# Regenerator/dpf-nets

Hardware: AMD Instinct MI355X
Metric: points/sec through 14-layer flow + Chamfer, B=32 N=2048 (higher is better)
Workload: dtype f16x3 MFMA operands, fp32 accumulate/points; 1 GPU; configs[1]: airplane autoencoder shapes, B=32 N=2048 per GPU: 14 coupling layers (first 14 of LocalCondRNVPDecoder(n_flows=5)), direct/eval-BN, + nn_distance both directions + CD reduction; clouds_per_gpu=32, points_per_cloud=2048, hidden=64, latent=128, global_clouds=32, per_layer_lists=False, launch=hipGraph replay, 10 step(s) per graph, steps_in_flight=1, settle_steps=400, parallelism=clouds sharded, no collective, sclk_mhz=2199, chamfer_impl=auto (matrix-core filtered exact search at this size)

## Files before the change

dpf_nets_amd/csrc/chamfer_mfma.hip:

```cpp
#include <hip/hip_runtime.h>
#include <limits.h>
#include <stdint.h>
#include <stdlib.h>

#include "dpf_hip.h"
#include "lds_attr.h"
#include "zero_fill.h"
#include "nn_refscan.h"

#pragma clang fp contract(off)

namespace {

typedef __bf16 bf16x8 __attribute__((ext_vector_type(8)));
typedef float f32x16 __attribute__((ext_vector_type(16)));
typedef uint32_t u32x4 __attribute__((ext_vector_type(4)));

constexpr int CT = 64;
constexpr int PROW = 100;
constexpr int SCH = 32;
constexpr int WCAP = SCH * 64 / 8;
constexpr int NNM_PTS = CT * 1024, NNM_LISTS = NNM_PTS + CT * PROW * 4;
__host__ __device__ constexpr int nnm_lds_bytes(int qw) { return NNM_LISTS + qw * SCH * 64 + qw * WCAP * 2; }

__device__ __forceinline__ uint32_t f2u(float x) { return __builtin_bit_cast(uint32_t, x); }
__device__ __forceinline__ float u2f(uint32_t x) { return __builtin_bit_cast(float, x); }
__device__ __forceinline__ uint32_t bf16_rne(float x) {
    const uint32_t u = f2u(x);
    return (u + 0x7FFFu + ((u >> 16) & 1u)) >> 16;
}
__device__ __forceinline__ void split2(float x, uint32_t &hi, uint32_t &lo) {
    const uint32_t h = f2u(x) & 0xFFFF0000u;
    hi = h >> 16;
    lo = bf16_rne(x - u2f(h));
}

__host__ __device__ inline int tiles_of(int n) { return (n + 31) / 32; }

__device__ __forceinline__ void cand_coord(float c, uint32_t &w0, uint32_t &w1) {
    uint32_t hi, lo;
    split2(c, hi, lo);
    w0 = hi | (hi << 16);
    w1 = lo | (lo << 16);
}
__device__ __forceinline__ void cand_fragment(float x, float y, float z, bool live, uint4 &h0, uint4 &h1) {
    cand_coord(x, h0.x, h0.y);
    cand_coord(y, h0.z, h0.w);
    cand_coord(z, h1.x, h1.y);
    const float w = (x * x + y * y) + z * z;
    const float ww = live ? w : 3.0e38f;
    const uint32_t wh = f2u(ww) & 0xFFFF0000u;
    const float r1 = ww - u2f(wh);
    const uint32_t wm = f2u(r1) & 0xFFFF0000u;
    const float r2 = r1 - u2f(wm);
    h1.z = (wh >> 16) | (live ? wm : 0u);
    h1.w = live ? bf16_rne(r2) : 0u;
}
__device__ __forceinline__ uint4 query_fragment(float x, float y, float z, int h) {
    uint32_t ah, al, bh, bl;
    split2(-2.0f * (h ? z : x), ah, al);
    split2(-2.0f * y, bh, bl);
    uint4 o;
    o.x = ah | (al << 16); o.y = o.x;
    o.z = h ? 0x3F803F80u : (bh | (bl << 16));
    o.w = h ? 0x00003F80u : o.z;
    return o;
}

struct MDir {
    const float *q, *c;
    float *dist;
    int *idx;
    int nq, nc;
    long qstride, cstride;
};
struct MArgs { MDir d[2]; int pn2; float *part; unsigned *ticket; float *cd; };

__device__ __forceinline__ f32x16 mfma(uint4 a, uint4 b) {
    const f32x16 z = {0.f, 0.f, 0.f, 0.f, 0.f, 0.f, 0.f, 0.f, 0.f, 0.f, 0.f, 0.f, 0.f, 0.f, 0.f, 0.f};
    return __builtin_amdgcn_mfma_f32_32x32x16_bf16(__builtin_bit_cast(bf16x8, a), __builtin_bit_cast(bf16x8, b), z, 0, 0, 0);
}
__device__ __forceinline__ float tile_min(const f32x16 &s) {
    float m = fminf(fminf(s[0], s[1]), s[2]);
    m = fminf(fminf(m, s[3]), s[4]);   m = fminf(fminf(m, s[5]), s[6]);
    m = fminf(fminf(m, s[7]), s[8]);   m = fminf(fminf(m, s[9]), s[10]);
    m = fminf(fminf(m, s[11]), s[12]); m = fminf(fminf(m, s[13]), s[14]);
    return fminf(fminf(m, s[15]), s[0]);
}
__device__ __forceinline__ float dist3(float cx, float cy, float cz, float qx, float qy, float qz) {
    const float dx = cx - qx, dy = cy - qy, dz = cz - qz;
    return (dx * dx + dy * dy) + dz * dz;
}
template <class P>
__device__ __forceinline__ void exact_tile(P cp, int nc, int t, int tl, int h, float qx, float qy, float qz,
                                           float &best, int &bidx) {
    float d[16];
#pragma unroll
    for (int g = 0; g < 4; ++g) {
        const float *row = cp + (size_t)tl * PROW + 8 * g + 4 * h;
        const float4 vx = *(const float4 *)row, vy = *(const float4 *)(row + 32), vz = *(const float4 *)(row + 64);
        d[4 * g + 0] = dist3(vx.x, vy.x, vz.x, qx, qy, qz); d[4 * g + 1] = dist3(vx.y, vy.y, vz.y, qx, qy, qz);
        d[4 * g + 2] = dist3(vx.z, vy.z, vz.z, qx, qy, qz); d[4 * g + 3] = dist3(vx.w, vy.w, vz.w, qx, qy, qz);
    }
    float m = fminf(fminf(d[0], d[1]), d[2]);
#pragma unroll
    for (int r = 3; r < 15; r += 2) m = fminf(fminf(m, d[r]), d[r + 1]);
    m = fminf(m, d[15]);
    if (m <= best) {
        int kmin = INT_MAX;
#pragma unroll
        for (int r = 15; r >= 0; --r) {
            const int k = t * 32 + 8 * (r >> 2) + 4 * h + (r & 3);
            kmin = (d[r] == m && k < nc) ? k : kmin;
        }
        const bool better = kmin != INT_MAX && (m < best || kmin < bidx);
        best = better ? m : best;
        bidx = better ? kmin : bidx;
    }
}

template <class P>
__device__ __forceinline__ void exact_tile_mk(P cp, int nc, int t, int tl, int h, float qx, float qy, float qz, float &m, int &kmin) {
    float d[16];
#pragma unroll
    for (int g = 0; g < 4; ++g) {
        const float *row = cp + (size_t)tl * PROW + 8 * g + 4 * h;
        const float4 vx = *(const float4 *)row, vy = *(const float4 *)(row + 32), vz = *(const float4 *)(row + 64);
        d[4 * g + 0] = dist3(vx.x, vy.x, vz.x, qx, qy, qz); d[4 * g + 1] = dist3(vx.y, vy.y, vz.y, qx, qy, qz);
        d[4 * g + 2] = dist3(vx.z, vy.z, vz.z, qx, qy, qz); d[4 * g + 3] = dist3(vx.w, vy.w, vz.w, qx, qy, qz);
    }
    m = fminf(fminf(d[0], d[1]), d[2]);
#pragma unroll
    for (int r = 3; r < 15; r += 2) m = fminf(fminf(m, d[r]), d[r + 1]);
    m = fminf(m, d[15]);
    kmin = INT_MAX;
#pragma unroll
    for (int r = 15; r >= 0; --r) {
        const int k = t * 32 + 8 * (r >> 2) + 4 * h + (r & 3);
        kmin = (d[r] == m && k < nc) ? k : kmin;
    }
}

typedef __attribute__((address_space(3))) void lds_void;
typedef __attribute__((address_space(1))) const void glb_void;

template <int QW>
__global__ __launch_bounds__(QW * 64) void nnm_kernel(MArgs args) {
    extern __shared__ __attribute__((aligned(16))) uint8_t lds[];
    uint4 *sfrag = (uint4 *)lds;
    float *spts = (float *)(lds + NNM_PTS);
    unsigned char *qtile = (unsigned char *)(lds + NNM_LISTS);
    __shared__ float s_r2[QW];
    const bool pairwise = args.pn2 > 0;
    const int dir = pairwise ? (int)(blockIdx.z & 1) : (int)blockIdx.z;
    const MDir A = args.d[dir];
    const int pi = pairwise ? (int)(blockIdx.z >> 1) : 0, pj = (int)blockIdx.y;
    const int bi = pairwise ? 0 : (int)blockIdx.y;
    const int nq = A.nq, nc = A.nc;
    const bool sums = args.part != nullptr;
    const size_t part_at = pairwise ? (((size_t)pi * args.pn2 + pj) * 2 + dir) * gridDim.x + blockIdx.x
                                    : ((size_t)bi * 2 + dir) * gridDim.x + blockIdx.x;
    const size_t unit = pairwise ? (size_t)pi * args.pn2 + pj : (size_t)bi;
    auto publish = [&](float t) {
        if (args.ticket == nullptr) { args.part[part_at] = t; return; }
        __hip_atomic_store(&args.part[part_at], t, __ATOMIC_RELAXED, __HIP_MEMORY_SCOPE_AGENT);
        asm volatile("s_waitcnt vmcnt(0)" ::: "memory");
        const unsigned nwg2 = 2u * gridDim.x;
        const unsigned old = __hip_atomic_fetch_add(&args.ticket[unit], 1u, __ATOMIC_RELAXED, __HIP_MEMORY_SCOPE_AGENT);
        if (old == nwg2 - 1) {
            const float *p = args.part + unit * nwg2;
            float s1 = 0.f, s2 = 0.f;
            for (unsigned x = 0; x < gridDim.x; ++x) {
                s1 += __hip_atomic_load(&p[x], __ATOMIC_RELAXED, __HIP_MEMORY_SCOPE_AGENT);
                s2 += __hip_atomic_load(&p[gridDim.x + x], __ATOMIC_RELAXED, __HIP_MEMORY_SCOPE_AGENT);
            }
            args.cd[unit] = s1 / (float)args.d[0].nq + s2 / (float)args.d[1].nq;
            __hip_atomic_store(&args.ticket[unit], 0u, __ATOMIC_RELAXED, __HIP_MEMORY_SCOPE_AGENT);
        }
    };
    if ((int)blockIdx.x * QW * 32 >= nq) {
        if (sums && threadIdx.x == 0) publish(0.f);
        return;
    }
    const int tid = threadIdx.x, lane = tid & 63, h = lane >> 5;
    const int wave = __builtin_amdgcn_readfirstlane(tid >> 6);
    const int qt = blockIdx.x * QW + wave;
    const int nqt = tiles_of(nq), nct = tiles_of(nc);
    const bool wave_live = qt < nqt;
    const size_t qcloud = pairwise ? (size_t)(dir == 0 ? pi : pj) * A.qstride : (size_t)bi * A.qstride;
    const size_t ccloud = pairwise ? (size_t)(dir == 0 ? pj : pi) * A.cstride : (size_t)bi * A.cstride;
    const float *__restrict__ cpts = A.c + ccloud;
    const int j = qt * 32 + (lane & 31);
    const float *qsrc = A.q + qcloud + (size_t)min(j, nq - 1) * 3;
    const float qx = qsrc[0], qy = qsrc[1], qz = qsrc[2];
    float mux, muy, muz;
    {
        const float *src = cpts + (size_t)min(lane, nc - 1) * 3;
        mux = src[0]; muy = src[1]; muz = src[2];
        for (int d = 32; d > 0; d >>= 1) { mux += __shfl_xor(mux, d); muy += __shfl_xor(muy, d); muz += __shfl_xor(muz, d); }
        mux *= 0.015625f; muy *= 0.015625f; muz *= 0.015625f;
    }
    const float qcx = qx - mux, qcy = qy - muy, qcz = qz - muz;
    const uint4 bq = query_fragment(qcx, qcy, qcz, h);
    const float INF_ = __builtin_inff();
    float r2 = j < nq ? (qcx * qcx + qcy * qcy) + qcz * qcz : 0.f;
    r2 = nn_not_finite(r2) ? INF_ : r2;
    if (nct > CT)
        for (int p = tid; p < nc; p += QW * 64) {
            const float *src = cpts + (size_t)p * 3;
            const float x = src[0] - mux, y = src[1] - muy, z = src[2] - muz;
            const float cn = (x * x + y * y) + z * z;
            r2 = nn_not_finite(cn) ? INF_ : fmaxf(r2, cn);
        }
    float tau = 0.f;
    bool slow = false;

    unsigned short *wl = (unsigned short *)(lds + NNM_LISTS + QW * SCH * 64) + (size_t)wave * WCAP;
    uint2 *res = (uint2 *)(qtile + (size_t)wave * SCH * 64);
    float smin = __builtin_inff();
    float best = __builtin_inff();
    int bidx = INT_MAX;
    const int npass = (nct + CT - 1) / CT;
    for (int pass = 0; pass < npass; ++pass) {
        const int t0 = pass * CT, tn = min(CT, nct - t0);
        if (pass > 0) __syncthreads();
        int tidp = tid;
        asm volatile("" : "+v"(tidp));
#pragma unroll
        for (int k = 0; k < CT * 32 / (QW * 64); ++k) {
            const int pl = tidp + k * QW * 64, t = pl >> 5, i = pl & 31, p = t0 * 32 + pl;
            if (t < tn) {
                const bool live = p < nc;
                float x = 0.f, y = 0.f, z = 0.f;
                if (live) { const float *src = cpts + (size_t)p * 3; x = src[0]; y = src[1]; z = src[2]; }
                uint4 f0, f1;
                const float cx = live ? x - mux : 0.f, cy = live ? y - muy : 0.f, cz = live ? z - muz : 0.f;
                cand_fragment(cx, cy, cz, live, f0, f1);
                sfrag[t * 64 + i] = f0;
                sfrag[t * 64 + 32 + i] = f1;
                spts[t * PROW + i] = live ? x : 3.0e38f; spts[t * PROW + 32 + i] = live ? y : 3.0e38f; spts[t * PROW + 64 + i] = live ? z : 3.0e38f;
                if (pass == 0) {
                    const float cn = (cx * cx + cy * cy) + cz * cz;
                    r2 = nn_not_finite(cn) ? INF_ : fmaxf(r2, cn);
                }
            }
        }
        if (pass == 0) {
            for (int d = 32; d > 0; d >>= 1) r2 = fmaxf(r2, __shfl_xor(r2, d));
            if (lane == 0) s_r2[wave] = r2;
        }
        __syncthreads();
        if (pass == 0) {
            float m = s_r2[0];
#pragma unroll
            for (int w = 1; w < QW; ++w) m = fmaxf(m, s_r2[w]);
            tau = m * 2.44140625e-4f;
            if (nn_not_finite(m)) { slow = true; break; }
        }
        if (wave_live) {
            for (int c0 = 0; c0 < tn; c0 += SCH) {
                const int cn = min(SCH, tn - c0);
                float mt[SCH];
                if (cn == SCH) {
                    const uint4 *fr = sfrag + c0 * 64 + lane;
                    if constexpr (QW < 16) {
                        uint4 fa = fr[0], fb = fr[64];
                        f32x16 a = mfma(fa, bq);
                        fa = fr[2 * 64];
#pragma unroll
                        for (int u = 0; u < SCH; u += 2) {
                            const f32x16 b = mfma(fb, bq);
                            if (u + 3 < SCH) fb = fr[(u + 3) * 64];
                            __builtin_amdgcn_sched_barrier(0);
                            mt[u] = tile_min(a);
                            __builtin_amdgcn_sched_barrier(0);
                            if (u + 2 < SCH) {
                                a = mfma(fa, bq);
                                if (u + 4 < SCH) fa = fr[(u + 4) * 64];
                            }
                            __builtin_amdgcn_sched_barrier(0);
                            mt[u + 1] = tile_min(b);
                            __builtin_amdgcn_sched_barrier(0);
                        }
                    } else {
                        f32x16 a = mfma(fr[0], bq);
#pragma unroll
                        for (int u = 0; u < SCH; u += 2) {
                            const f32x16 b = mfma(fr[(u + 1) * 64], bq);
                            __builtin_amdgcn_sched_barrier(0);
                            mt[u] = tile_min(a);
                            __builtin_amdgcn_sched_barrier(0);
                            if (u + 2 < SCH) a = mfma(fr[(u + 2) * 64], bq);
                            __builtin_amdgcn_sched_barrier(0);
                            mt[u + 1] = tile_min(b);
                            __builtin_amdgcn_sched_barrier(0);
                        }
                    }
                } else {
                    auto frag = [&](int u) { return sfrag[(c0 + min(u, cn - 1)) * 64 + lane]; };
                    f32x16 a = mfma(frag(0), bq);
#pragma unroll
                    for (int u = 0; u < SCH; u += 2) {
                        const f32x16 b = mfma(frag(u + 1), bq);
                        __builtin_amdgcn_sched_barrier(0);
                        mt[u] = tile_min(a);
                        __builtin_amdgcn_sched_barrier(0);
                        if (u + 2 < SCH) a = mfma(frag(u + 2), bq);
                        __builtin_amdgcn_sched_barrier(0);
                        mt[u + 1] = tile_min(b);
                        __builtin_amdgcn_sched_barrier(0);
                    }
                }
                float cm = fminf(fminf(mt[0], mt[1]), mt[2]);
#pragma unroll
                for (int u = 3; u + 1 < SCH; u += 2) cm = fminf(fminf(cm, mt[u]), mt[u + 1]);
                cm = fminf(cm, mt[SCH - 1]);
                smin = fminf(smin, cm);
                const float thr = fminf(smin, __shfl_xor(smin, 32)) + tau;
                unsigned smask = 0;
#pragma unroll
                for (int u = 0; u < SCH; ++u)
                    asm("v_cmp_le_f32 vcc, %1, %2\n\tv_addc_co_u32 %0, vcc, %0, %0, vcc" : "+v"(smask) : "v"(mt[u]), "v"(thr) : "vcc");
                if (cn < SCH) smask &= ~0u << (SCH - cn);
                const int nsurv = __builtin_popcount(smask);
                int smax = nsurv;
                for (int d = 32; d > 0; d >>= 1) smax = max(smax, __shfl_xor(smax, d));
                smax = __builtin_amdgcn_readfirstlane(smax);
                int off = nsurv;
#pragma unroll
                for (int d = 1; d < 64; d <<= 1) { const int v = __shfl_up(off, d); off += lane >= d ? v : 0; }
                const int W = __builtin_amdgcn_readlane(off, 63);
                off -= nsurv;
                if (W <= WCAP) {
                    {
                        unsigned mk = smask;
                        for (int e = 0; e < smax; ++e) {
                            if (mk != 0) wl[off + e] = (unsigned short)((lane << 8) | (SCH - 1 - __builtin_ctz(mk)));
                            mk &= mk - 1;
                        }
                    }
                    __builtin_amdgcn_fence(__ATOMIC_RELEASE, "wavefront");
                    __builtin_amdgcn_wave_barrier();
                    for (int i0 = 0; i0 < W; i0 += 64) {
                        const int i = i0 + lane;
                        const unsigned item = wl[min(i, W - 1)];
                        const int sl = (int)(item >> 8), tl = c0 + (int)(item & 255u);
                        const float sx = __shfl(qx, sl), sy = __shfl(qy, sl), sz = __shfl(qz, sl);
                        float m; int k;
                        exact_tile_mk(spts, nc, t0 + tl, tl, sl >> 5, sx, sy, sz, m, k);
                        if (i < W) res[i] = make_uint2(__float_as_uint(m), (unsigned)k);
                    }
                    __builtin_amdgcn_fence(__ATOMIC_RELEASE, "wavefront");
                    __builtin_amdgcn_wave_barrier();
                    for (int e = 0; e < smax; ++e) {
                        if (e < nsurv) {
                            const uint2 r = res[off + e];
                            const float m = __uint_as_float(r.x);
                            const int k = (int)r.y;
                            const bool better = k != INT_MAX && (m < best || (m == best && k < bidx));
                            best = better ? m : best;
                            bidx = better ? k : bidx;
                        }
                    }
                    __builtin_amdgcn_fence(__ATOMIC_RELEASE, "wavefront");
                    __builtin_amdgcn_wave_barrier();
                } else {
                    unsigned mk = smask;
                    for (int e = 0; e < smax; ++e) {
                        const bool take = mk != 0;
                        const int tl = c0 + (take ? SCH - 1 - __builtin_ctz(mk) : 0);
                        mk &= mk - 1;
                        float b2 = best; int i2 = bidx;
                        exact_tile(spts, nc, t0 + tl, tl, h, qx, qy, qz, b2, i2);
                        if (take) { best = b2; bidx = i2; }
                    }
                }
            }
        }
    }
    if (slow && wave_live)
        nn_reference_scan(cpts, nc, qx, qy, qz, best, bidx);
    if (!wave_live && !sums) return;
    const float od = __shfl_xor(best, 32);
    const int oi = __shfl_xor(bidx, 32);
    if (od < best || (od == best && oi < bidx)) { best = od; bidx = oi; }
    int tid_out = threadIdx.x;
    asm volatile("" : "+v"(tid_out));
    const int j_out = (blockIdx.x * QW + (tid_out >> 6)) * 32 + (tid_out & 31);
    if (!pairwise) {
        if (wave_live && h == 0 && j_out < nq) {
            A.dist[(size_t)bi * nq + j_out] = best;
            A.idx[(size_t)bi * nq + j_out] = bidx;
        }
        if (!sums) return;
    }
    float sum = (wave_live && h == 0 && j_out < nq) ? best : 0.f;
    for (int d = 16; d > 0; d >>= 1) sum += __shfl_xor(sum, d);
    __syncthreads();
    if (lane == 0) s_r2[wave] = sum;
    __syncthreads();
    if (tid == 0) {
        float t = s_r2[0];
#pragma unroll
        for (int w = 1; w < QW; ++w) t += s_r2[w];
        publish(t);
    }
}

__global__ __launch_bounds__(64) void nnm_surrogate_kernel(const float *__restrict__ q, int nq, const float *__restrict__ c, int nc,
                                                           float *__restrict__ s, float *__restrict__ out3) {
    __shared__ uint4 frag[64];
    const int lane = threadIdx.x, h = lane >> 5, i = lane & 31, qt = blockIdx.x, ct = blockIdx.y;
    float mux, muy, muz;
    {
        const float *src = c + (size_t)min(lane, nc - 1) * 3;
        mux = src[0]; muy = src[1]; muz = src[2];
        for (int d = 32; d > 0; d >>= 1) { mux += __shfl_xor(mux, d); muy += __shfl_xor(muy, d); muz += __shfl_xor(muz, d); }
        mux *= 0.015625f; muy *= 0.015625f; muz *= 0.015625f;
    }
    const int j = qt * 32 + i, p = ct * 32 + i;
    const float *qsrc = q + (size_t)min(j, nq - 1) * 3;
    const uint4 bq = query_fragment(qsrc[0] - mux, qsrc[1] - muy, qsrc[2] - muz, h);
    if (h == 0) {
        const bool live = p < nc;
        const float *src = c + (size_t)min(p, nc - 1) * 3;
        uint4 f0, f1;
        cand_fragment(live ? src[0] - mux : 0.f, live ? src[1] - muy : 0.f, live ? src[2] - muz : 0.f, live, f0, f1);
        frag[i] = f0; frag[32 + i] = f1;
    }
    __syncthreads();
    const f32x16 a = mfma(frag[lane], bq);
#pragma unroll
    for (int r = 0; r < 16; ++r) {
        const int k = ct * 32 + 8 * (r >> 2) + 4 * h + (r & 3);
        if (j < nq && k < nc) s[(size_t)j * nc + k] = a[r];
    }
    if (qt == 0 && ct == 0) {
        float r2 = 0.f;
#pragma clang loop vectorize(disable) interleave(disable)
        for (int t = lane; t < nq + nc; t += 64) {
            const float *src = t < nq ? q + (size_t)t * 3 : c + (size_t)(t - nq) * 3;
            const float x = src[0] - mux, y = src[1] - muy, z = src[2] - muz;
            r2 = fmaxf(r2, (x * x + y * y) + z * z);
        }
        for (int d = 32; d > 0; d >>= 1) r2 = fmaxf(r2, __shfl_xor(r2, d));
        if (lane == 0) { out3[0] = mux; out3[1] = muy; out3[2] = muz; out3[3] = r2; }
    }
}

}

extern "C" int dpf_debug_nn_surrogate(int nq, const float *q, int nc, const float *c, float *s, float *out4, dpf_stream_t stream) {
    if (nq <= 0 || nc <= 0 || !q || !c || !s || !out4) return DPF_EINVAL;
    hipLaunchKernelGGL(nnm_surrogate_kernel, dim3(tiles_of(nq), tiles_of(nc)), dim3(64), 0, (hipStream_t)stream, q, nq, c, nc, s, out4);
    return (int)hipGetLastError();
}

extern "C" size_t dpf_nndistance_mfma_workspace_bytes(int b, int n, int m) {
    (void)b; (void)n; (void)m;
    return 0;
}

static long nnm_workgroups(int b, int n, int m, int qw) {
    return (long)b * ((n + qw * 32 - 1) / (qw * 32) + (m + qw * 32 - 1) / (qw * 32));
}

template <int QW>
static int launch_nnm_qw(const MArgs &ma, int b, int nmax, hipStream_t s) {
    const int lds = nnm_lds_bytes(QW);
    static LdsLimit limit;
    if (hipError_t e = limit.ensure((const void *)nnm_kernel<QW>, lds); e != hipSuccess) return (int)e;
    hipLaunchKernelGGL(nnm_kernel<QW>, dim3((nmax + QW * 32 - 1) / (QW * 32), b, 2), dim3(QW * 64), lds, s, ma);
    return (int)hipGetLastError();
}

static int launch_nnm(int b, int n, const float *xyz, long xyz_stride, int m, const float *xyz2, long xyz2_stride,
                      float *result, int *result_i, float *result2, int *result2_i, hipStream_t s, float *part = nullptr,
                      bool force16 = false, unsigned *ticket = nullptr, float *cd = nullptr) {
    MArgs ma;
    ma.pn2 = 0; ma.part = part; ma.ticket = ticket; ma.cd = cd;
    ma.d[0] = MDir{xyz, xyz2, result, result_i, n, m, xyz_stride, xyz2_stride};
    ma.d[1] = MDir{xyz2, xyz, result2, result2_i, m, n, xyz2_stride, xyz_stride};
    const int nmax = n > m ? n : m;
    static const int qw_env = getenv("DPF_NNM_QW") ? atoi(getenv("DPF_NNM_QW")) : 0;
    if (force16 || qw_env == 16) return launch_nnm_qw<16>(ma, b, nmax, s);
    if (qw_env == 8) return launch_nnm_qw<8>(ma, b, nmax, s);
    if (qw_env == 4) return launch_nnm_qw<4>(ma, b, nmax, s);
    if (nnm_workgroups(b, n, m, 16) >= 128) return launch_nnm_qw<16>(ma, b, nmax, s);
    return nnm_workgroups(b, n, m, 8) >= 128 ? launch_nnm_qw<8>(ma, b, nmax, s) : launch_nnm_qw<4>(ma, b, nmax, s);
}

bool nn_small_serves(int b, int n, int m);
static bool nnm_pays(int b, int n, int m) {
    if (b <= 0 || n <= 0 || m <= 0 || b > 65535 || n > 65535 * 32 || m > 65535 * 32) return false;
    if (nnm_workgroups(b, n, m, 8) < 64) return false;
    const double pairs = 2.0 * (double)b * (double)n * (double)m;
    if (pairs >= 1.0e8) return true;
    return pairs >= 3.0e7 && (n > m ? n : m) <= CT * 32 && !nn_small_serves(b, n, m);
}

extern "C" int dpf_nndistance_mfma(int b, int n, const float *xyz, int m, const float *xyz2, float *result,
                                   int *result_i, float *result2, int *result2_i, void *workspace,
                                   size_t workspace_bytes, dpf_stream_t stream) {
    (void)workspace; (void)workspace_bytes;
    if (b < 0 || n <= 0 || m <= 0) return DPF_EINVAL;
    if (b == 0) return 0;
    if (!xyz || !xyz2 || !result || !result_i || !result2 || !result2_i) return DPF_EINVAL;
    if (b > 65535 || n > 65535 * 32 || m > 65535 * 32 || (n < 32 && m < 32))
        return dpf_nndistance(b, n, xyz, m, xyz2, result, result_i, result2, result2_i, stream);
    return launch_nnm(b, n, xyz, (long)n * 3, m, xyz2, (long)m * 3, result, result_i, result2, result2_i, (hipStream_t)stream);
}

extern "C" int dpf_nndistance_auto(int b, int n, const float *xyz, int m, const float *xyz2, float *result, int *result_i,
                                   float *result2, int *result2_i, dpf_stream_t stream) {
    if (xyz && xyz2 && result && result_i && result2 && result2_i && nnm_pays(b, n, m))
        return launch_nnm(b, n, xyz, (long)n * 3, m, xyz2, (long)m * 3, result, result_i, result2, result2_i, (hipStream_t)stream);
    return dpf_nndistance(b, n, xyz, m, xyz2, result, result_i, result2, result2_i, stream);
}

extern "C" int dpf_nndistance_strided_auto(int b, int n, const float *xyz, long xyz_stride, int m, const float *xyz2,
                                           long xyz2_stride, float *result, int *result_i, float *result2, int *result2_i,
                                           dpf_stream_t stream) {
    if (xyz && xyz2 && result && result_i && result2 && result2_i && xyz_stride >= 0 && xyz2_stride >= 0 && nnm_pays(b, n, m))
        return launch_nnm(b, n, xyz, xyz_stride, m, xyz2, xyz2_stride, result, result_i, result2, result2_i, (hipStream_t)stream);
    return dpf_nndistance_strided(b, n, xyz, xyz_stride, m, xyz2, xyz2_stride, result, result_i, result2, result2_i, stream);
}

static int pairwise_qw(int nmax) { return nmax <= 256 ? 8 : 16; }
extern "C" size_t dpf_pairwise_cd_workspace_bytes(int n1, int n2, int n, int m) {
    const int nmax = n > m ? n : m, per = pairwise_qw(nmax) * 32;
    return (size_t)n1 * n2 * (2 * ((nmax + per - 1) / per) + 1) * sizeof(float);
}
extern "C" int dpf_pairwise_cd(int n1, int n2, int n, int m, const float *clouds1, const float *clouds2, float *cds,
                               void *workspace, size_t workspace_bytes, dpf_stream_t stream) {
    if (n1 < 0 || n2 < 0 || n <= 0 || m <= 0) return DPF_EINVAL;
    if (n1 == 0 || n2 == 0) return 0;
    if (!clouds1 || !clouds2 || !cds || !workspace) return DPF_EINVAL;
    if (workspace_bytes < dpf_pairwise_cd_workspace_bytes(n1, n2, n, m)) return DPF_EINVAL;
    if (n2 > 65535 || n1 > 32767 || n < 32 || m < 32 || n > 65535 * 32 || m > 65535 * 32) return DPF_ENOSUP;
    MArgs ma;
    ma.d[0] = MDir{clouds1, clouds2, nullptr, nullptr, n, m, (long)n * 3, (long)m * 3};
    ma.d[1] = MDir{clouds2, clouds1, nullptr, nullptr, m, n, (long)m * 3, (long)n * 3};
    const int nmax = n > m ? n : m, qw = pairwise_qw(nmax), nwg = (nmax + qw * 32 - 1) / (qw * 32);
    const long npairs = (long)n1 * n2;
    hipStream_t s = (hipStream_t)stream;
    ma.pn2 = n2; ma.ticket = (unsigned *)workspace; ma.part = (float *)workspace + npairs; ma.cd = cds;
    if (hipError_t e = dpf_zero_async(workspace, (size_t)npairs * sizeof(unsigned), s); e != hipSuccess) return (int)e;
    if (qw == 16) {
        const int lds = nnm_lds_bytes(16);
        static LdsLimit limit;
        if (hipError_t e = limit.ensure((const void *)nnm_kernel<16>, lds); e != hipSuccess) return (int)e;
        hipLaunchKernelGGL(nnm_kernel<16>, dim3(nwg, n2, 2 * n1), dim3(16 * 64), lds, s, ma);
    } else {
        const int lds = nnm_lds_bytes(8);
        static LdsLimit limit;
        if (hipError_t e = limit.ensure((const void *)nnm_kernel<8>, lds); e != hipSuccess) return (int)e;
        hipLaunchKernelGGL(nnm_kernel<8>, dim3(nwg, n2, 2 * n1), dim3(8 * 64), lds, s, ma);
    }
    return (int)hipGetLastError();
}

extern "C" size_t dpf_nndistance_cd_workspace_bytes(int b, int n, int m) {
    const int nmax = n > m ? n : m;
    return (size_t)(b > 0 ? b : 0) * (2 * ((nmax + 63) / 64) + 1) * sizeof(float) + 16;
}
int nn_small_cd(int b, int n, const float *xyz, int m, const float *xyz2, float *result, int *result_i, float *result2,
                int *result2_i, float *cd, void *workspace, int tickets_are_zero, hipStream_t s);
extern "C" int dpf_nndistance_cd(int b, int n, const float *xyz, int m, const float *xyz2, float *result, int *result_i,
                                 float *result2, int *result2_i, float *cd, void *workspace, size_t workspace_bytes,
                                 int tickets_are_zero, dpf_stream_t stream) {
    if (b < 0 || n <= 0 || m <= 0) return DPF_EINVAL;
    if (b == 0) return 0;
    if (!xyz || !xyz2 || !result || !result_i || !result2 || !result2_i || !cd) return DPF_EINVAL;
    hipStream_t s = (hipStream_t)stream;
    if (workspace && workspace_bytes >= dpf_nndistance_cd_workspace_bytes(b, n, m) && nnm_pays(b, n, m)) {
        if (!tickets_are_zero)
            if (hipError_t e = dpf_zero_async(workspace, (size_t)b * sizeof(unsigned), s); e != hipSuccess) return (int)e;
        return launch_nnm(b, n, xyz, (long)n * 3, m, xyz2, (long)m * 3, result, result_i, result2, result2_i, s,
                          (float *)workspace + b, false, (unsigned *)workspace, cd);
    }
    if (workspace && workspace_bytes >= dpf_nndistance_cd_workspace_bytes(b, n, m) && !nnm_pays(b, n, m)) {
        const int rc = nn_small_cd(b, n, xyz, m, xyz2, result, result_i, result2, result2_i, cd, workspace, tickets_are_zero, s);
        if (rc != DPF_ENOSUP) return rc;
    }
    int rc = dpf_nndistance_auto(b, n, xyz, m, xyz2, result, result_i, result2, result2_i, stream);
    if (rc) return rc;
    return dpf_chamfer_reduce(b, n, m, result, result2, cd, stream);
}
```

Baseline: 926.4 million points/s.

## Prefetch first candidate pass into registers and streamline nnm wave reductions

The Chamfer matrix-core kernel now loads the first pass of candidate points into registers before the mean and radius setup, so those global loads overlap that work. The first-pass LDS staging moves out of the loop, and the slow path skips the loop instead of breaking out of it. Several smaller changes ride along: DPP-based wave scan and max replace shuffle loops, ballot-driven loop bounds replace the wave max, the survivor-mask asm is batched, argmin selection is simplified, the final reduction uses a separate shared buffer to drop one barrier, and the ticket reduction is unrolled. It also adds optional DPF_PROFILE timestamp instrumentation that compiles away by default, at the cost of more register pressure from the prefetch arrays.

```diff
diff --git a/dpf_nets_amd/csrc/chamfer_mfma.hip b/dpf_nets_amd/csrc/chamfer_mfma.hip
--- a/dpf_nets_amd/csrc/chamfer_mfma.hip
+++ b/dpf_nets_amd/csrc/chamfer_mfma.hip
@@ -74,7 +74,12 @@
     int nq, nc;
     long qstride, cstride;
 };
-struct MArgs { MDir d[2]; int pn2; float *part; unsigned *ticket; float *cd; };
+struct MArgs {
+    MDir d[2]; int pn2; float *part; unsigned *ticket; float *cd;
+#ifdef DPF_PROFILE
+    unsigned long long *prof;
+#endif
+};
 
 __device__ __forceinline__ f32x16 mfma(uint4 a, uint4 b) {
     const f32x16 z = {0.f, 0.f, 0.f, 0.f, 0.f, 0.f, 0.f, 0.f, 0.f, 0.f, 0.f, 0.f, 0.f, 0.f, 0.f, 0.f};
@@ -133,13 +138,37 @@
 #pragma unroll
     for (int r = 3; r < 15; r += 2) m = fminf(fminf(m, d[r]), d[r + 1]);
     m = fminf(m, d[15]);
-    kmin = INT_MAX;
-#pragma unroll
-    for (int r = 15; r >= 0; --r) {
-        const int k = t * 32 + 8 * (r >> 2) + 4 * h + (r & 3);
-        kmin = (d[r] == m && k < nc) ? k : kmin;
-    }
-}
+    int rmin = 16;
+#pragma unroll
+    for (int r = 15; r >= 0; --r) rmin = d[r] == m ? r : rmin;
+    const int k = t * 32 + 8 * (rmin >> 2) + 4 * h + (rmin & 3);
+    kmin = (rmin < 16 && k < nc) ? k : INT_MAX;
+}
+
+template <int CTRL, int ROW_MASK = 0xF>
+__device__ __forceinline__ unsigned dpp_or0(unsigned v) {
+    return (unsigned)__builtin_amdgcn_update_dpp(0, (int)v, CTRL, ROW_MASK, 0xF, true);
+}
+__device__ __forceinline__ unsigned wave_scan_add(unsigned v) {
+    v += dpp_or0<0x111>(v); v += dpp_or0<0x112>(v); v += dpp_or0<0x114>(v); v += dpp_or0<0x118>(v);
+    v += dpp_or0<0x142, 0xA>(v);
+    v += dpp_or0<0x143, 0xC>(v);
+    return v;
+}
+__device__ __forceinline__ unsigned wave_max_u32(unsigned v) {
+    v = max(v, dpp_or0<0x111>(v)); v = max(v, dpp_or0<0x112>(v)); v = max(v, dpp_or0<0x114>(v)); v = max(v, dpp_or0<0x118>(v));
+    v = max(v, dpp_or0<0x142, 0xA>(v));
+    v = max(v, dpp_or0<0x143, 0xC>(v));
+    return (unsigned)__builtin_amdgcn_readlane((int)v, 63);
+}
+
+#ifdef DPF_PROFILE
+#define DPF_T(i) { __builtin_amdgcn_sched_barrier(0); \
+    if (prof_at != nullptr) { const unsigned long long t_ = __builtin_amdgcn_s_memtime(); if ((threadIdx.x & 63) == 0) prof_at[i] = t_; } \
+    __builtin_amdgcn_sched_barrier(0); }
+#else
+#define DPF_T(i)
+#endif
 
 typedef __attribute__((address_space(3))) void lds_void;
 typedef __attribute__((address_space(1))) const void glb_void;
@@ -147,10 +176,8 @@
 template <int QW>
 __global__ __launch_bounds__(QW * 64) void nnm_kernel(MArgs args) {
     extern __shared__ __attribute__((aligned(16))) uint8_t lds[];
-    uint4 *sfrag = (uint4 *)lds;
-    float *spts = (float *)(lds + NNM_PTS);
     unsigned char *qtile = (unsigned char *)(lds + NNM_LISTS);
-    __shared__ float s_r2[QW];
+    __shared__ float s_r2[QW], s_sum[QW];
     const bool pairwise = args.pn2 > 0;
     const int dir = pairwise ? (int)(blockIdx.z & 1) : (int)blockIdx.z;
     const MDir A = args.d[dir];
@@ -170,9 +197,17 @@
         if (old == nwg2 - 1) {
             const float *p = args.part + unit * nwg2;
             float s1 = 0.f, s2 = 0.f;
-            for (unsigned x = 0; x < gridDim.x; ++x) {
-                s1 += __hip_atomic_load(&p[x], __ATOMIC_RELAXED, __HIP_MEMORY_SCOPE_AGENT);
-                s2 += __hip_atomic_load(&p[gridDim.x + x], __ATOMIC_RELAXED, __HIP_MEMORY_SCOPE_AGENT);
+            for (unsigned x0 = 0; x0 < gridDim.x; x0 += 4) {
+                float v1[4], v2[4];
+#pragma unroll
+                for (unsigned u = 0; u < 4; ++u) {
+                    const unsigned x = min(x0 + u, gridDim.x - 1);
+                    v1[u] = __hip_atomic_load(&p[x], __ATOMIC_RELAXED, __HIP_MEMORY_SCOPE_AGENT);
+                    v2[u] = __hip_atomic_load(&p[gridDim.x + x], __ATOMIC_RELAXED, __HIP_MEMORY_SCOPE_AGENT);
+                }
+#pragma unroll
+                for (unsigned u = 0; u < 4; ++u)
+                    if (x0 + u < gridDim.x) { s1 += v1[u]; s2 += v2[u]; }
             }
             args.cd[unit] = s1 / (float)args.d[0].nq + s2 / (float)args.d[1].nq;
             __hip_atomic_store(&args.ticket[unit], 0u, __ATOMIC_RELAXED, __HIP_MEMORY_SCOPE_AGENT);
@@ -184,6 +219,12 @@
     }
     const int tid = threadIdx.x, lane = tid & 63, h = lane >> 5;
     const int wave = __builtin_amdgcn_readfirstlane(tid >> 6);
+#ifdef DPF_PROFILE
+    unsigned long long *prof_at = nullptr;
+    if (args.prof != nullptr && blockIdx.y < 2 && blockIdx.z == 0 && gridDim.x <= 4)
+        prof_at = args.prof + ((size_t)(blockIdx.y * gridDim.x + blockIdx.x) * QW + wave) * 16;
+#endif
+    DPF_T(0)
     const int qt = blockIdx.x * QW + wave;
     const int nqt = tiles_of(nq), nct = tiles_of(nc);
     const bool wave_live = qt < nqt;
@@ -193,6 +234,15 @@
     const int j = qt * 32 + (lane & 31);
     const float *qsrc = A.q + qcloud + (size_t)min(j, nq - 1) * 3;
     const float qx = qsrc[0], qy = qsrc[1], qz = qsrc[2];
+    constexpr int KPT = CT * 32 / (QW * 64);
+    const int npass = (nct + CT - 1) / CT;
+    float px[KPT], py[KPT], pz[KPT];
+#pragma unroll
+    for (int k = 0; k < KPT; ++k) {
+        const int p = tid + k * QW * 64;
+        px[k] = 0.f; py[k] = 0.f; pz[k] = 0.f;
+        if (p < nc) { const float *src = cpts + (size_t)p * 3; px[k] = src[0]; py[k] = src[1]; pz[k] = src[2]; }
+    }
     float mux, muy, muz;
     {
         const float *src = cpts + (size_t)min(lane, nc - 1) * 3;
@@ -205,6 +255,7 @@
     const float INF_ = __builtin_inff();
     float r2 = j < nq ? (qcx * qcx + qcy * qcy) + qcz * qcz : 0.f;
     r2 = nn_not_finite(r2) ? INF_ : r2;
+    DPF_T(1)
     if (nct > CT)
         for (int p = tid; p < nc; p += QW * 64) {
             const float *src = cpts + (size_t)p * 3;
@@ -212,50 +263,69 @@
             const float cn = (x * x + y * y) + z * z;
             r2 = nn_not_finite(cn) ? INF_ : fmaxf(r2, cn);
         }
-    float tau = 0.f;
-    bool slow = false;
+
+    uint4 *sfrag = (uint4 *)lds;
+    float *spts = (float *)(lds + NNM_PTS);
+    auto put = [&](int pl, bool live, float x, float y, float z) {
+        const int t = pl >> 5, i = pl & 31;
+        uint4 f0, f1;
+        const float cx = live ? x - mux : 0.f, cy = live ? y - muy : 0.f, cz = live ? z - muz : 0.f;
+        cand_fragment(cx, cy, cz, live, f0, f1);
+        sfrag[t * 64 + i] = f0;
+        sfrag[t * 64 + 32 + i] = f1;
+        spts[t * PROW + i] = live ? x : 3.0e38f; spts[t * PROW + 32 + i] = live ? y : 3.0e38f; spts[t * PROW + 64 + i] = live ? z : 3.0e38f;
+        return (cx * cx + cy * cy) + cz * cz;
+    };
+    {
+        const int tn = min(CT, nct);
+        int tidp = tid;
+        asm volatile("" : "+v"(tidp));
+#pragma unroll
+        for (int k = 0; k < KPT; ++k) {
+            const int pl = tidp + k * QW * 64;
+            if ((pl >> 5) < tn) {
+                const float cn = put(pl, pl < nc, px[k], py[k], pz[k]);
+                r2 = nn_not_finite(cn) ? INF_ : fmaxf(r2, cn);
+            }
+        }
+    }
+    DPF_T(2)
+    const float r2w = u2f(wave_max_u32(f2u(r2)));
+    if (lane == 0) s_r2[wave] = r2w;
+    __syncthreads();
+    float tau;
+    bool slow;
+    {
+        float m = s_r2[0];
+#pragma unroll
+        for (int w = 1; w < QW; ++w) m = fmaxf(m, s_r2[w]);
+        tau = m * 2.44140625e-4f;
+        slow = nn_not_finite(m);
+    }
+    DPF_T(3)
 
     unsigned short *wl = (unsigned short *)(lds + NNM_LISTS + QW * SCH * 64) + (size_t)wave * WCAP;
     uint2 *res = (uint2 *)(qtile + (size_t)wave * SCH * 64);
     float smin = __builtin_inff();
     float best = __builtin_inff();
     int bidx = INT_MAX;
-    const int npass = (nct + CT - 1) / CT;
-    for (int pass = 0; pass < npass; ++pass) {
+    for (int pass = 0; pass < (slow ? 0 : npass); ++pass) {
         const int t0 = pass * CT, tn = min(CT, nct - t0);
-        if (pass > 0) __syncthreads();
-        int tidp = tid;
-        asm volatile("" : "+v"(tidp));
-#pragma unroll
-        for (int k = 0; k < CT * 32 / (QW * 64); ++k) {
-            const int pl = tidp + k * QW * 64, t = pl >> 5, i = pl & 31, p = t0 * 32 + pl;
-            if (t < tn) {
-                const bool live = p < nc;
-                float x = 0.f, y = 0.f, z = 0.f;
-                if (live) { const float *src = cpts + (size_t)p * 3; x = src[0]; y = src[1]; z = src[2]; }
-                uint4 f0, f1;
-                const float cx = live ? x - mux : 0.f, cy = live ? y - muy : 0.f, cz = live ? z - muz : 0.f;
-                cand_fragment(cx, cy, cz, live, f0, f1);
-                sfrag[t * 64 + i] = f0;
-                sfrag[t * 64 + 32 + i] = f1;
-                spts[t * PROW + i] = live ? x : 3.0e38f; spts[t * PROW + 32 + i] = live ? y : 3.0e38f; spts[t * PROW + 64 + i] = live ? z : 3.0e38f;
-                if (pass == 0) {
-                    const float cn = (cx * cx + cy * cy) + cz * cz;
-                    r2 = nn_not_finite(cn) ? INF_ : fmaxf(r2, cn);
+        if (pass > 0) {
+            __syncthreads();
+            int tidp = tid;
+            asm volatile("" : "+v"(tidp));
+#pragma unroll
+            for (int k = 0; k < KPT; ++k) {
+                const int pl = tidp + k * QW * 64, p = t0 * 32 + pl;
+                if ((pl >> 5) < tn) {
+                    const bool live = p < nc;
+                    float x = 0.f, y = 0.f, z = 0.f;
+                    if (live) { const float *src = cpts + (size_t)p * 3; x = src[0]; y = src[1]; z = src[2]; }
+                    put(pl, live, x, y, z);
                 }
             }
-        }
-        if (pass == 0) {
-            for (int d = 32; d > 0; d >>= 1) r2 = fmaxf(r2, __shfl_xor(r2, d));
-            if (lane == 0) s_r2[wave] = r2;
-        }
-        __syncthreads();
-        if (pass == 0) {
-            float m = s_r2[0];
-#pragma unroll
-            for (int w = 1; w < QW; ++w) m = fmaxf(m, s_r2[w]);
-            tau = m * 2.44140625e-4f;
-            if (nn_not_finite(m)) { slow = true; break; }
+            __syncthreads();
         }
         if (wave_live) {
             for (int c0 = 0; c0 < tn; c0 += SCH) {
@@ -311,6 +381,7 @@
                         __builtin_amdgcn_sched_barrier(0);
                     }
                 }
+                DPF_T(4 + 5 * (c0 / SCH))
                 float cm = fminf(fminf(mt[0], mt[1]), mt[2]);
 #pragma unroll
                 for (int u = 3; u + 1 < SCH; u += 2) cm = fminf(fminf(cm, mt[u]), mt[u + 1]);
@@ -318,27 +389,33 @@
                 smin = fminf(smin, cm);
                 const float thr = fminf(smin, __shfl_xor(smin, 32)) + tau;
                 unsigned smask = 0;
-#pragma unroll
-                for (int u = 0; u < SCH; ++u)
-                    asm("v_cmp_le_f32 vcc, %1, %2\n\tv_addc_co_u32 %0, vcc, %0, %0, vcc" : "+v"(smask) : "v"(mt[u]), "v"(thr) : "vcc");
+                static_assert(SCH == 32, "the mask is built sixteen tiles at a time, twice");
+#define NNM_MK(n) "v_cmp_le_f32 vcc, %" #n ", %17\n\tv_addc_co_u32 %0, vcc, %0, %0, vcc\n\t"
+#pragma unroll
+                for (int u = 0; u < SCH; u += 16)
+                    asm(NNM_MK(1) NNM_MK(2) NNM_MK(3) NNM_MK(4) NNM_MK(5) NNM_MK(6) NNM_MK(7) NNM_MK(8)
+                        NNM_MK(9) NNM_MK(10) NNM_MK(11) NNM_MK(12) NNM_MK(13) NNM_MK(14) NNM_MK(15) NNM_MK(16)
+                        : "+v"(smask)
+                        : "v"(mt[u]), "v"(mt[u + 1]), "v"(mt[u + 2]), "v"(mt[u + 3]), "v"(mt[u + 4]), "v"(mt[u + 5]), "v"(mt[u + 6]),
+                          "v"(mt[u + 7]), "v"(mt[u + 8]), "v"(mt[u + 9]), "v"(mt[u + 10]), "v"(mt[u + 11]), "v"(mt[u + 12]),
+                          "v"(mt[u + 13]), "v"(mt[u + 14]), "v"(mt[u + 15]), "v"(thr)
+                        : "vcc");
+#undef NNM_MK
                 if (cn < SCH) smask &= ~0u << (SCH - cn);
                 const int nsurv = __builtin_popcount(smask);
-                int smax = nsurv;
-                for (int d = 32; d > 0; d >>= 1) smax = max(smax, __shfl_xor(smax, d));
-                smax = __builtin_amdgcn_readfirstlane(smax);
-                int off = nsurv;
-#pragma unroll
-                for (int d = 1; d < 64; d <<= 1) { const int v = __shfl_up(off, d); off += lane >= d ? v : 0; }
+                DPF_T(5 + 5 * (c0 / SCH))
+                int off = (int)wave_scan_add((unsigned)nsurv);
                 const int W = __builtin_amdgcn_readlane(off, 63);
                 off -= nsurv;
                 if (W <= WCAP) {
                     {
                         unsigned mk = smask;
-                        for (int e = 0; e < smax; ++e) {
+                        for (int e = 0; __builtin_amdgcn_ballot_w64(mk != 0) != 0; ++e) {
                             if (mk != 0) wl[off + e] = (unsigned short)((lane << 8) | (SCH - 1 - __builtin_ctz(mk)));
                             mk &= mk - 1;
                         }
                     }
+                    DPF_T(6 + 5 * (c0 / SCH))
                     __builtin_amdgcn_fence(__ATOMIC_RELEASE, "wavefront");
                     __builtin_amdgcn_wave_barrier();
                     for (int i0 = 0; i0 < W; i0 += 64) {
@@ -352,7 +429,8 @@
                     }
                     __builtin_amdgcn_fence(__ATOMIC_RELEASE, "wavefront");
                     __builtin_amdgcn_wave_barrier();
-                    for (int e = 0; e < smax; ++e) {
+                    DPF_T(7 + 5 * (c0 / SCH))
+                    for (int e = 0; __builtin_amdgcn_ballot_w64(e < nsurv) != 0; ++e) {
                         if (e < nsurv) {
                             const uint2 r = res[off + e];
                             const float m = __uint_as_float(r.x);
@@ -364,7 +442,9 @@
                     }
                     __builtin_amdgcn_fence(__ATOMIC_RELEASE, "wavefront");
                     __builtin_amdgcn_wave_barrier();
+                    DPF_T(8 + 5 * (c0 / SCH))
                 } else {
+                    const int smax = (int)wave_max_u32((unsigned)nsurv);
                     unsigned mk = smask;
                     for (int e = 0; e < smax; ++e) {
                         const bool take = mk != 0;
@@ -394,17 +474,18 @@
         }
         if (!sums) return;
     }
+    DPF_T(14)
     float sum = (wave_live && h == 0 && j_out < nq) ? best : 0.f;
     for (int d = 16; d > 0; d >>= 1) sum += __shfl_xor(sum, d);
-    __syncthreads();
-    if (lane == 0) s_r2[wave] = sum;
+    if (lane == 0) s_sum[wave] = sum;
     __syncthreads();
     if (tid == 0) {
-        float t = s_r2[0];
-#pragma unroll
-        for (int w = 1; w < QW; ++w) t += s_r2[w];
+        float t = s_sum[0];
+#pragma unroll
+        for (int w = 1; w < QW; ++w) t += s_sum[w];
         publish(t);
     }
+    DPF_T(15)
 }
 
 __global__ __launch_bounds__(64) void nnm_surrogate_kernel(const float *__restrict__ q, int nq, const float *__restrict__ c, int nc,
@@ -461,6 +542,11 @@
     return 0;
 }
 
+#ifdef DPF_PROFILE
+static unsigned long long *g_nnm_prof = nullptr;
+extern "C" void dpf_debug_set_nnm_prof(void *p) { g_nnm_prof = (unsigned long long *)p; }
+#endif
+
 static long nnm_workgroups(int b, int n, int m, int qw) {
     return (long)b * ((n + qw * 32 - 1) / (qw * 32) + (m + qw * 32 - 1) / (qw * 32));
 }
@@ -479,6 +565,9 @@
                       bool force16 = false, unsigned *ticket = nullptr, float *cd = nullptr) {
     MArgs ma;
     ma.pn2 = 0; ma.part = part; ma.ticket = ticket; ma.cd = cd;
+#ifdef DPF_PROFILE
+    ma.prof = g_nnm_prof;
+#endif
     ma.d[0] = MDir{xyz, xyz2, result, result_i, n, m, xyz_stride, xyz2_stride};
     ma.d[1] = MDir{xyz2, xyz, result2, result2_i, m, n, xyz2_stride, xyz_stride};
     const int nmax = n > m ? n : m;
@@ -545,6 +634,9 @@
     const long npairs = (long)n1 * n2;
     hipStream_t s = (hipStream_t)stream;
     ma.pn2 = n2; ma.ticket = (unsigned *)workspace; ma.part = (float *)workspace + npairs; ma.cd = cds;
+#ifdef DPF_PROFILE
+    ma.prof = nullptr;
+#endif
     if (hipError_t e = dpf_zero_async(workspace, (size_t)npairs * sizeof(unsigned), s); e != hipSuccess) return (int)e;
     if (qw == 16) {
         const int lds = nnm_lds_bytes(16);
```

After: 944.2 million points/s (median of 6 runs). 1.9% higher.
